# nacho-pancho/binary-image-compression

Measured on AMD Instinct MI355X. Metric: encode MPixels/s (and MB/s out) at 1/2/4/8 GPUs; bit-exact vs CPU, higher is better.
Workload: dtype u64; 1 GPU; c3: 16384x16384 8-bit gray -> 8 bitplanes -> med -> per-row runs -> Golomb + EG streams per plane (bitplanes formed in registers, not returned: planes NULL) -- the count pass writes the EG stream, the Golomb emission reads the residual rows from it; rows=16384, cols=16384, planes_per_gpu=8, parallelism=dp1 (independent images per GPU)

## Files before the change

binary-image-compression_amd/csrc/bic_kernels.hip:

```cpp
#include "bic_device.h"
#include "bic_k1pi.h"
#include "bic_kstat.h"

namespace bic {

__device__ __forceinline__ uint64_t transpose8x8(uint64_t x) {
  uint64_t t;
  t = (x ^ (x >> 7)) & 0x00AA00AA00AA00AAull;
  x = x ^ t ^ (t << 7);
  t = (x ^ (x >> 14)) & 0x0000CCCC0000CCCCull;
  x = x ^ t ^ (t << 14);
  t = (x ^ (x >> 28)) & 0x00000000F0F0F0F0ull;
  x = x ^ t ^ (t << 28);
  return x;
}

template <bool VEC, bool GC, int SP = 0>
__global__ __launch_bounds__(kBlock) void k_bitplanes_u8(const uint8_t* __restrict__ gray, size_t pitch,
                                                         uint32_t rows, uint32_t cols, uint32_t used,
                                                         int plane0, int nplanes, uint64_t* __restrict__ planes,
                                                         uint32_t wpr) {
  const uint32_t groups = (used + 63) / 64;
  const uint64_t gw = (uint64_t)blockIdx.x * kWaves + wave_id();
  if (gw >= (uint64_t)rows * groups) return;
// ... 206 lines not shown
  auto load = [&](uint32_t row, uint64_t (&v)[LW]) {
    const uint64_t* src = pl + (uint64_t)row * g.wpr + w0;
    if constexpr (LW == 1) {
      v[0] = w0 < g.used ? src[0] : 0;
    } else {
#pragma unroll
      for (int i = 0; i < LW; i += 2) {
        ulonglong2 t = make_ulonglong2(0, 0);
        if (w0 + i < g.used) t = *reinterpret_cast<const ulonglong2*>(src + i);
        v[i] = t.x;
        v[i + 1] = t.y;
      }
    }
  };
  uint64_t up[LW], cur[LW];
#pragma unroll
  for (int i = 0; i < LW; ++i) up[i] = 0;
  if (PREDICT && r0) load(r0 - 1, up);
  load(r0, cur);
  const uint32_t nr = min((uint32_t)RPW, g.rows - r0);
  for (uint32_t r = 0; r < nr; ++r) {
    const uint32_t row = r0 + r;
    uint64_t nxt[LW];
    if (r + 1 < nr) load(row + 1, nxt);
    LaneK k;
    uint64_t D[LW];
#pragma unroll
    for (int i = 0; i < LW; ++i) D[i] = PREDICT ? cur[i] ^ up[i] : cur[i];
    const uint64_t dl = wave_shr1_u64(D[LW - 1]);
#pragma unroll
    for (int i = 0; i < LW; ++i) {
      const uint32_t w = w0 + i;
      uint64_t R = D[i];
      if constexpr (PREDICT) {
        R = D[i] ^ ((D[i] >> 1) | ((i ? D[i - 1] : dl) << 63));
        if (row == 0 && w == 0) R &= ~BIC_MSB;
      }
      R = w < g.used ? (w == g.used - 1 ? R & g.trail : R) : 0;
      lanek_word(k, R, (int32_t)(w * 64));
      up[i] = cur[i];
    }
    const uint64_t id = (uint64_t)plane * g.rows + row;
    lanek_store(k, krec + id, kpos + id, sones + id);
#pragma unroll
    for (int i = 0; i < LW; ++i) cur[i] = nxt[i];
  }
}

template <int CTRL>
__device__ __forceinline__ int dpp16(int old, int v) {
  return __builtin_amdgcn_update_dpp(old, v, CTRL, 0xf, 0xf, false);
}
__device__ __forceinline__ uint32_t row16_incl_sum(uint32_t x) {
  x += (uint32_t)dpp16<0x111>(0, (int)x);
  x += (uint32_t)dpp16<0x112>(0, (int)x);
  x += (uint32_t)dpp16<0x114>(0, (int)x);
  x += (uint32_t)dpp16<0x118>(0, (int)x);
  return x;
}
__device__ __forceinline__ int row16_incl_max(int x) {
  x = max(x, dpp16<0x111>(INT_MIN, x));
  x = max(x, dpp16<0x112>(INT_MIN, x));
  x = max(x, dpp16<0x114>(INT_MIN, x));
  x = max(x, dpp16<0x118>(INT_MIN, x));
  return x;
}
__device__ __forceinline__ int row16_max(int x) {
  x = max(x, dpp16<0xB1>(x, x));
  x = max(x, dpp16<0x4E>(x, x));
  x = max(x, dpp16<0x141>(x, x));
  x = max(x, dpp16<0x140>(x, x));
  return x;
}
__device__ __forceinline__ int row16_min(int x) {
  x = min(x, dpp16<0xB1>(x, x));
  x = min(x, dpp16<0x4E>(x, x));
  x = min(x, dpp16<0x141>(x, x));
  x = min(x, dpp16<0x140>(x, x));
  return x;
}
__device__ __forceinline__ uint32_t row16_sum(uint32_t x) {
  x += (uint32_t)dpp16<0xB1>(0, (int)x);
  x += (uint32_t)dpp16<0x4E>(0, (int)x);
  x += (uint32_t)dpp16<0x141>(0, (int)x);
  x += (uint32_t)dpp16<0x140>(0, (int)x);
  return x;
}

template <int RPW, bool PREDICT, bool V16>
__global__ __launch_bounds__(kBlock) void k_med_kstat16(Geom g, const uint64_t* __restrict__ planes,
                                                        uint32_t* __restrict__ sones, int4* __restrict__ krec,
                                                        uint32_t* __restrict__ kpos, uint32_t* __restrict__ zero) {
  if (blockIdx.x == 0 && threadIdx.x < kZeroWords) zero[threadIdx.x] = 0;
  const int lane = lane_id(), q = lane & 15, grp = lane >> 4;
  const uint32_t wpp = (g.rows + RPW - 1) / RPW;
  const uint64_t gw = (uint64_t)xcd_remap(blockIdx.x, gridDim.x) * kWaves + wave_id();
  if (gw >= (uint64_t)wpp * g.nplanes) return;
  const uint32_t plane = (uint32_t)(gw / wpp), r0 = (uint32_t)(gw % wpp) * RPW;
  const uint64_t* pl = planes + (uint64_t)plane * g.plane_words;
  const uint32_t w0 = 4 * (uint32_t)q;
  const uint32_t nr = min((uint32_t)RPW, g.rows - r0);
  auto load = [&](uint32_t rb, uint64_t (&P)[4], uint64_t (&U)[4]) {
    const uint32_t rr = rb + (uint32_t)grp < nr ? r0 + rb + (uint32_t)grp : r0;
    if constexpr (V16) {
      const uint32_t wc = w0 < g.used ? w0 : 0;
      const ulonglong2* p2 = reinterpret_cast<const ulonglong2*>(pl + (uint64_t)rr * g.wpr + wc);
      const ulonglong2 a = p2[0], b = p2[1];
      P[0] = a.x; P[1] = a.y; P[2] = b.x; P[3] = b.y;
      if (PREDICT && rr) {
        const ulonglong2* u2 = reinterpret_cast<const ulonglong2*>(pl + (uint64_t)(rr - 1) * g.wpr + wc);
        const ulonglong2 c = u2[0], d = u2[1];
        U[0] = c.x; U[1] = c.y; U[2] = d.x; U[3] = d.y;
      } else {
        U[0] = U[1] = U[2] = U[3] = 0;
      }
      return;
    }
#pragma unroll
    for (int i = 0; i < 4; ++i) {
      const uint32_t w = w0 + i, wc = w < g.used ? w : g.used - 1;
      P[i] = pl[(uint64_t)rr * g.wpr + wc];
      U[i] = (PREDICT && rr) ? pl[(uint64_t)(rr - 1) * g.wpr + wc] : 0ull;
    }
  };
  uint64_t P[4], U[4];
  load(0, P, U);
  for (uint32_t rb = 0; rb < nr; rb += 4) {
    const uint32_t row = r0 + rb + (uint32_t)grp;
    const bool in = rb + (uint32_t)grp < nr;
    const uint32_t rr = in ? row : r0;
    uint64_t NP[4], NU[4];
    if (rb + 4 < nr) load(rb + 4, NP, NU);
    uint64_t D[4];
#pragma unroll
    for (int i = 0; i < 4; ++i) D[i] = P[i] ^ U[i];
    const uint64_t dl = ((uint64_t)(uint32_t)dpp16<0x111>(0, (int)(uint32_t)(D[3] >> 32)) << 32) |
                        (uint32_t)dpp16<0x111>(0, (int)(uint32_t)D[3]);
    LaneK k;
#pragma unroll
    for (int i = 0; i < 4; ++i) {
      const uint32_t w = w0 + i;
      uint64_t R = D[i];
      if constexpr (PREDICT) {
        R = D[i] ^ ((D[i] >> 1) | ((i ? D[i - 1] : dl) << 63));
        if (rr == 0 && w == 0) R &= ~BIC_MSB;
      }
      R = w < g.used ? (w == g.used - 1 ? R & g.trail : R) : 0;
      lanek_word(k, R, (int32_t)(w * 64));
    }
    const uint32_t inc = row16_incl_sum(k.ones);
    const int32_t base = (int32_t)(inc - k.ones);
    const int mx = row16_incl_max(k.last);
    const int32_t before = dpp16<0x111>(-1, mx);
    uint32_t chg = k.chg;
    int32_t first = -1;
    if (k.ones) {
      if (before >= 0) chg += (uint32_t)((before ^ k.first) & 1);
      else first = k.first;
    }
    const int32_t q0 = row16_max(k.ones ? k.q0 - 2 * base : -kNoOnes);
    const int32_t qh = row16_max(k.ones ? k.qh - 3 * base : -kNoOnes);
    const int32_t ql = row16_min(k.ones ? k.ql - 2 * base : kNoOnes);
    const uint32_t c = row16_sum(chg);
    const int32_t f = row16_max(first);
    const uint32_t tot = row16_sum(k.ones);
    const int32_t last = row16_max(k.last);
    if (q == 0 && in) {
      const uint64_t id = (uint64_t)plane * g.rows + row;
      krec[id] = make_int4(q0, qh, ql, (int32_t)(tot | (c << 16)));
      kpos[id] = ((uint32_t)f & 0xffffu) | ((uint32_t)last << 16);
      sones[id] = tot;
    }
#pragma unroll
    for (int i = 0; i < 4; ++i) {
      P[i] = NP[i];
      U[i] = NU[i];
    }
  }
}

void launch_row_ones(hipStream_t s, const Geom& g, const uint64_t* planes, int predict, uint32_t* sones,
                     int4* krec, uint32_t* kpos, uint32_t* zero) {
  constexpr int RPW = 8;
  const uint32_t wpp = (g.rows + RPW - 1) / RPW;
  const uint32_t grid = (uint32_t)(((uint64_t)wpp * g.nplanes + kWaves - 1) / kWaves);
#define BIC_KST(LW, P) k_med_kstat<LW, RPW, P><<<grid, kBlock, 0, s>>>(g, planes, sones, krec, kpos, zero)
  if (g.used <= 64) {
    constexpr int R16 = 16;
    const uint32_t wpp16 = (g.rows + R16 - 1) / R16;
    const uint32_t grid16 = (uint32_t)(((uint64_t)wpp16 * g.nplanes + kWaves - 1) / kWaves);
    const bool v16 = g.wpr % 4 == 0 && g.used % 4 == 0 && reinterpret_cast<uintptr_t>(planes) % 16 == 0;
#define BIC_K16(P, V) k_med_kstat16<R16, P, V><<<grid16, kBlock, 0, s>>>(g, planes, sones, krec, kpos, zero)
    if (predict) { if (v16) BIC_K16(true, true); else BIC_K16(true, false); }
    else { if (v16) BIC_K16(false, true); else BIC_K16(false, false); }
#undef BIC_K16
  }
  else if (g.used <= 128) { if (predict) BIC_KST(2, true); else BIC_KST(2, false); }
  else { if (predict) BIC_KST(4, true); else BIC_KST(4, false); }
#undef BIC_KST
}

template <int LW, int RPW, bool PREDICT>
__global__ __launch_bounds__(kBlock) void k_pbm_kstat(Geom g, const uint8_t* __restrict__ raster, uint64_t stride,
                                                      uint64_t* __restrict__ dst, int store_r,
                                                      uint32_t* __restrict__ sones, int4* __restrict__ krec,
                                                      uint32_t* __restrict__ kpos, uint32_t* __restrict__ zero) {
  static_assert(LW % 2 == 0, "a lane stores 16-byte word pairs");
  if (blockIdx.x == 0 && threadIdx.x < kZeroWords) zero[threadIdx.x] = 0;
  const int lane = lane_id();
  const uint32_t wpp = (g.rows + RPW - 1) / RPW;
  const uint64_t gw = (uint64_t)xcd_remap(blockIdx.x, gridDim.x) * kWaves + wave_id();
  if (gw >= (uint64_t)wpp * g.nplanes) return;
  const uint32_t plane = (uint32_t)(gw / wpp), r0 = (uint32_t)(gw % wpp) * RPW;
  const uint32_t nb = (g.cols + 7) / 8;
  const uint8_t* fp = raster + (uint64_t)plane * stride;
  const uint64_t fb = reinterpret_cast<uint64_t>(fp);
  const uint64_t lastc = (fb + (uint64_t)g.rows * nb - 1) & ~7ull;
  const uint32_t w0 = LW * lane;
  auto load = [&](uint32_t row, uint64_t (&v)[LW]) {
    const uint64_t a = fb + (uint64_t)row * nb + 8ull * w0;
    const uint32_t sh = 8 * (uint32_t)__builtin_amdgcn_readfirstlane((int)((fb + (uint64_t)row * nb) & 7));
    const uint64_t ca = a & ~7ull;
    uint64_t c[LW + 1];
#pragma unroll
    for (int j = 0; j <= LW; ++j) {
      const bool need = w0 + (j ? j - 1 : 0) < g.used && (j < LW || sh) && ca + 8 * j <= lastc;
      c[j] = need ? *reinterpret_cast<const uint64_t*>(fp + (int64_t)(ca + 8 * j - fb)) : 0ull;
    }
#pragma unroll
    for (int i = 0; i < LW; ++i) {
      const uint32_t w = w0 + i;
      const uint64_t x = bswap64(sh ? (c[i] >> sh) | (c[i + 1] << (64 - sh)) : c[i]);
      v[i] = w < g.used ? (w == g.used - 1 ? x & g.trail : x) : 0;
    }
  };
  uint64_t up[LW], cur[LW];
#pragma unroll
  for (int i = 0; i < LW; ++i) up[i] = 0;
  if (PREDICT && r0) load(r0 - 1, up);
  load(r0, cur);
  const uint32_t nr = min((uint32_t)RPW, g.rows - r0);
  uint64_t* out = dst + (uint64_t)plane * g.plane_words;
  for (uint32_t r = 0; r < nr; ++r) {
    const uint32_t row = r0 + r;
    uint64_t nxt[LW];
    if (r + 1 < nr) load(row + 1, nxt);
    LaneK k;
    uint64_t D[LW], R[LW];
#pragma unroll
    for (int i = 0; i < LW; ++i) D[i] = PREDICT ? cur[i] ^ up[i] : cur[i];
    const uint64_t dl = wave_shr1_u64(D[LW - 1]);
#pragma unroll
    for (int i = 0; i < LW; ++i) {
      const uint32_t w = w0 + i;
      R[i] = D[i];
      if constexpr (PREDICT) {
        R[i] = D[i] ^ ((D[i] >> 1) | ((i ? D[i - 1] : dl) << 63));
        if (row == 0 && w == 0) R[i] &= ~BIC_MSB;
      }
      R[i] = w < g.used ? (w == g.used - 1 ? R[i] & g.trail : R[i]) : 0;
      lanek_word(k, R[i], (int32_t)(w * 64));
      up[i] = cur[i];
    }
    const uint64_t id = (uint64_t)plane * g.rows + row;
    lanek_store(k, krec + id, kpos + id, sones + id);
    uint64_t* orow = out + (uint64_t)row * g.wpr;
#pragma unroll
    for (int i = 0; i < LW; i += 2)
      if (w0 + i < g.wpr)
        *reinterpret_cast<ulonglong2*>(orow + w0 + i) =
            store_r ? make_ulonglong2(R[i], R[i + 1]) : make_ulonglong2(cur[i], cur[i + 1]);
    for (uint32_t w = 64 * LW + 2 * lane; w < g.wpr; w += 128)
      *reinterpret_cast<ulonglong2*>(orow + w) = make_ulonglong2(0, 0);
#pragma unroll
    for (int i = 0; i < LW; ++i) cur[i] = nxt[i];
  }
}

void launch_pbm_rows(hipStream_t s, const uint8_t* raster, uint64_t stride, const Geom& g, int predict, uint64_t* dst,
                     bool store_resid, uint32_t* sones, int4* krec, uint32_t* kpos, uint32_t* zero) {
  constexpr int RPW = 8;
  const uint32_t wpp = (g.rows + RPW - 1) / RPW;
  const uint32_t grid = (uint32_t)(((uint64_t)wpp * g.nplanes + kWaves - 1) / kWaves);
  const int sr = store_resid && predict ? 1 : 0;
#define BIC_PKS(LW, P) k_pbm_kstat<LW, RPW, P><<<grid, kBlock, 0, s>>>(g, raster, stride, dst, sr, sones, krec, kpos, zero)
  if (g.used <= 128) { if (predict) BIC_PKS(2, true); else BIC_PKS(2, false); }
  else { if (predict) BIC_PKS(4, true); else BIC_PKS(4, false); }
#undef BIC_PKS
}

#ifndef BIC_GRAY_ROWS
#define BIC_GRAY_ROWS 4
#endif
#ifndef BIC_GRAY_ROWS_BM
#define BIC_GRAY_ROWS_BM 1
#endif
constexpr int kGrayRowsP = BIC_GRAY_ROWS, kGrayRowsBM = BIC_GRAY_ROWS_BM;
uint32_t gray_strips(const Geom& g) { return (g.used + 63) / 64; }

__device__ __forceinline__ void perm_t4(uint32_t w0, uint32_t w1, uint32_t w2, uint32_t w3, uint32_t (&out)[4]) {
  const uint32_t a01 = __builtin_amdgcn_perm(w0, w1, 0x04000501u), b01 = __builtin_amdgcn_perm(w0, w1, 0x06020703u);
  const uint32_t a23 = __builtin_amdgcn_perm(w2, w3, 0x04000501u), b23 = __builtin_amdgcn_perm(w2, w3, 0x06020703u);
  out[0] = __builtin_amdgcn_perm(a01, a23, 0x07060302u);
  out[1] = __builtin_amdgcn_perm(a01, a23, 0x05040100u);
  out[2] = __builtin_amdgcn_perm(b01, b23, 0x07060302u);
  out[3] = __builtin_amdgcn_perm(b01, b23, 0x05040100u);
}

__device__ __forceinline__ uint64_t transpose8x8_bs(uint32_t x0, uint32_t x1) {
  uint32_t hi = __builtin_bswap32(x0), lo = __builtin_bswap32(x1);
  uint32_t t;
  t = __builtin_amdgcn_bitop3_b32(lo, lo >> 7, 0x00AA00AAu, 0x28);
  lo = __builtin_amdgcn_bitop3_b32(lo, t, t << 7, 0x96);
  t = __builtin_amdgcn_bitop3_b32(hi, hi >> 7, 0x00AA00AAu, 0x28);
  hi = __builtin_amdgcn_bitop3_b32(hi, t, t << 7, 0x96);
  t = __builtin_amdgcn_bitop3_b32(lo, lo >> 14, 0x0000CCCCu, 0x28);
  lo = __builtin_amdgcn_bitop3_b32(lo, t, t << 14, 0x96);
  t = __builtin_amdgcn_bitop3_b32(hi, hi >> 14, 0x0000CCCCu, 0x28);
  hi = __builtin_amdgcn_bitop3_b32(hi, t, t << 14, 0x96);
  t = __builtin_amdgcn_bitop3_b32(lo, hi << 4, 0xF0F0F0F0u, 0x28);
  lo ^= t;
  hi ^= t >> 4;
  return ((uint64_t)hi << 32) | lo;
}

template <bool FULL = false>
__device__ __forceinline__ void gray_to_planes(const uint4 (&v)[4], uint64_t (&pw)[8], uint64_t mask) {
  uint64_t T[8];
#pragma unroll
  for (int i = 0; i < 4; ++i) {
    T[2 * i] = transpose8x8_bs(v[i].x, v[i].y);
    T[2 * i + 1] = transpose8x8_bs(v[i].z, v[i].w);
  }
  uint32_t XL[4], YL[4], XH[4], YH[4];
  perm_t4((uint32_t)T[0], (uint32_t)T[1], (uint32_t)T[2], (uint32_t)T[3], XL);
  perm_t4((uint32_t)T[4], (uint32_t)T[5], (uint32_t)T[6], (uint32_t)T[7], YL);
  perm_t4((uint32_t)(T[0] >> 32), (uint32_t)(T[1] >> 32), (uint32_t)(T[2] >> 32), (uint32_t)(T[3] >> 32), XH);
  perm_t4((uint32_t)(T[4] >> 32), (uint32_t)(T[5] >> 32), (uint32_t)(T[6] >> 32), (uint32_t)(T[7] >> 32), YH);
#pragma unroll
  for (int b = 0; b < 4; ++b) {
    pw[b] = ((uint64_t)XL[b] << 32) | YL[b];
    pw[4 + b] = ((uint64_t)XH[b] << 32) | YH[b];
    if constexpr (!FULL) {
      pw[b] &= mask;
      pw[4 + b] &= mask;
    }
  }
}

#ifndef BIC_GRAY_PREFETCH
#define BIC_GRAY_PREFETCH 1
#endif
constexpr bool kGrayPrefetch = BIC_GRAY_PREFETCH != 0;
#ifndef BIC_GRAY_BYTEMED
#define BIC_GRAY_BYTEMED 1
#endif
constexpr bool kGrayByteMed = BIC_GRAY_BYTEMED != 0;
template <bool PREDICT, bool STORE_R>
constexpr int gray_rows_per_wave() { return kGrayByteMed && PREDICT && STORE_R ? kGrayRowsBM : kGrayRowsP; }
__device__ __forceinline__ void load64_mis(const uint8_t* src, uint4 (&v)[4]) {
  const uintptr_t a = reinterpret_cast<uintptr_t>(src);
  const uint32_t mis = (uint32_t)(a & 15), bs = mis & 3, dq = mis >> 2;
  const uint4* b = reinterpret_cast<const uint4*>(src - mis);
  uint32_t in[20];
#pragma unroll
  for (int q = 0; q < 4; ++q) {
    const uint4 x = b[q];
    in[4 * q] = x.x;
    in[4 * q + 1] = x.y;
    in[4 * q + 2] = x.z;
    in[4 * q + 3] = x.w;
  }
  const uint4 x4 = mis ? b[4] : make_uint4(0, 0, 0, 0);
  in[16] = x4.x;
  in[17] = x4.y;
  in[18] = x4.z;
  in[19] = x4.w;
#define BIC_MIS_CASE(DQ)                                                                                    \
  case DQ:                                                                                                  \
    _Pragma("unroll") for (int q = 0; q < 4; ++q) v[q] =                                                    \
        make_uint4(__builtin_amdgcn_alignbyte(in[4 * q + DQ + 1], in[4 * q + DQ], bs),                     \
                   __builtin_amdgcn_alignbyte(in[4 * q + DQ + 2], in[4 * q + DQ + 1], bs),                 \
                   __builtin_amdgcn_alignbyte(in[4 * q + DQ + 3], in[4 * q + DQ + 2], bs),                 \
                   __builtin_amdgcn_alignbyte(in[4 * q + DQ + 4], in[4 * q + DQ + 3], bs));                \
    break;
  switch (dq) {
    BIC_MIS_CASE(0)
    BIC_MIS_CASE(1)
    BIC_MIS_CASE(2)
    default: BIC_MIS_CASE(3)
  }
#undef BIC_MIS_CASE
}

__device__ __forceinline__ void gray4(uint4 (&v)[4]) {
#pragma unroll
  for (int q = 0; q < 4; ++q)
    v[q] = make_uint4(v[q].x ^ ((v[q].x >> 1) & 0x7f7f7f7fu), v[q].y ^ ((v[q].y >> 1) & 0x7f7f7f7fu),
                      v[q].z ^ ((v[q].z >> 1) & 0x7f7f7f7fu), v[q].w ^ ((v[q].w >> 1) & 0x7f7f7f7fu));
}

struct Raw16 {
  uint4 cur[8], up[8];
};

template <bool PREDICT, bool FULL, bool STORE_R, bool NP8, bool EGS, bool MIS = false, int S16 = 0, bool GC = false,
          int CT = 0, int SP = 0>
__device__ __forceinline__ void gray_strip_rows(const uint8_t* __restrict__ gray, size_t pitch, const Geom& g,
                                                uint32_t ns, uint32_t s, uint32_t r0, uint32_t plane0,
                                                uint64_t* __restrict__ planes, uint32_t* __restrict__ sones,
                                                int4* __restrict__ krec, uint32_t* __restrict__ kpos, uint32_t* tw,
                                                uint64_t* __restrict__ out_e, uint64_t eg_stride, uint32_t bo = 0,
                                                const Raw16* pre = nullptr, uint32_t lo16 = 0) {
  const int lane = lane_id();
  const int np = NP8 ? 8 : (int)g.nplanes;
  const uint32_t w = s * 64 + lane;
  const bool in = FULL || w < g.used;
  const uint64_t mask = FULL ? ~0ull : in ? (w == g.used - 1 ? g.trail : ~0ull) : 0ull;
  auto load = [&](uint32_t row, uint4 (&v)[4], uint32_t& lb) {
    const uint8_t* src = gray + (uint64_t)row * pitch + (uint64_t)w * (S16 == 3 ? 192 : S16 ? 128 : 64);
    if constexpr (S16 == 3) {
      uint4 c[12];
      if (in) {
        if constexpr (MIS) {
#pragma unroll
          for (int t = 0; t < 3; ++t) {
            uint4 a[4];
            load64_mis(src + 64 * t, a);
#pragma unroll
            for (int q = 0; q < 4; ++q) c[4 * t + q] = a[q];
          }
        } else {
#pragma unroll
          for (int q = 0; q < 12; ++q) c[q] = reinterpret_cast<const uint4*>(src)[q];
        }
      } else {
#pragma unroll
        for (int q = 0; q < 12; ++q) c[q] = make_uint4(0, 0, 0, 0);
      }
      const uint32_t s1 = rgb_sel1(bo), s2 = rgb_sel2(bo);
      auto pick = [&](uint32_t d0, uint32_t d1, uint32_t d2) {
        uint32_t x = rgb_pick4(d0, d1, d2, s1, s2);
        if constexpr (CT != 0)
          if (bo != 1) x = ct_forward4<CT>(x, rgb_pick4(d0, d1, d2, rgb_sel1(1), rgb_sel2(1)));
        if constexpr (GC) x ^= (x >> 1) & 0x7f7f7f7fu;
        return x;
      };
#pragma unroll
      for (int q = 0; q < 4; ++q)
        v[q] = make_uint4(pick(c[3 * q].x, c[3 * q].y, c[3 * q].z), pick(c[3 * q].w, c[3 * q + 1].x, c[3 * q + 1].y),
                          pick(c[3 * q + 1].z, c[3 * q + 1].w, c[3 * q + 2].x),
                          pick(c[3 * q + 2].y, c[3 * q + 2].z, c[3 * q + 2].w));
    } else if constexpr (S16) {
      uint4 c[8];
      if constexpr (S16 == 2) {
#pragma unroll
        for (int q = 0; q < 8; ++q) c[q] = row == r0 ? pre->cur[q] : pre->up[q];
      } else if (in) {
        if constexpr (MIS) {
          uint4 a[4], b[4];
          load64_mis(src, a);
          load64_mis(src + 64, b);
#pragma unroll
          for (int q = 0; q < 4; ++q) c[q] = a[q], c[4 + q] = b[q];
        } else {
#pragma unroll
          for (int q = 0; q < 8; ++q) c[q] = reinterpret_cast<const uint4*>(src)[q];
        }
      } else {
#pragma unroll
        for (int q = 0; q < 8; ++q) c[q] = make_uint4(0, 0, 0, 0);
      }
      const uint32_t sel = bo ? 0x07050301u : 0x06040200u;
      auto pick = [&](uint32_t hi2, uint32_t lo2) {
        uint32_t x = __builtin_amdgcn_perm(hi2, lo2, sel);
        if constexpr (GC) {
          x ^= (x >> 1) & 0x7f7f7f7fu;
          if (lo16) x ^= (__builtin_amdgcn_perm(hi2, lo2, sel ^ 0x01010101u) & 0x01010101u) << 7;
        }
        return x;
      };
#pragma unroll
      for (int q = 0; q < 4; ++q)
        v[q] = make_uint4(pick(c[2 * q].y, c[2 * q].x), pick(c[2 * q].w, c[2 * q].z), pick(c[2 * q + 1].y, c[2 * q + 1].x),
                          pick(c[2 * q + 1].w, c[2 * q + 1].z));
    } else if constexpr (MIS) {
      if (in) load64_mis(src, v);
      else
#pragma unroll
        for (int q = 0; q < 4; ++q) v[q] = make_uint4(0, 0, 0, 0);
    } else {
#pragma unroll
      for (int q = 0; q < 4; ++q) v[q] = in ? reinterpret_cast<const uint4*>(src)[q] : make_uint4(0, 0, 0, 0);
    }
    if constexpr (S16 == 3) lb = (lane == 0 && s > 0) ? (uint32_t)src[(int)bo - 3] : 0u;
    else if constexpr (S16) lb = (lane == 0 && s > 0) ? (uint32_t)src[(int)bo - 2] : 0u;
    else lb = (lane == 0 && s > 0) ? (uint32_t)src[-1] : 0u;
    if constexpr (S16 == 3 && CT != 0)
      if (bo != 1 && lane == 0 && s > 0) lb = ct_forward4<CT>(lb, (uint32_t)src[-2]) & 0xffu;
    if constexpr (SP != 0) {
      static_assert(S16 == 0 || SP == 0, "sample prediction: one-byte gray samples only");
      uint32_t prev = (uint32_t)__builtin_amdgcn_update_dpp(0, (int)v[3].w, 0x138, 0xf, 0xf, true);
      if (lane == 0) prev = lb << 24;
#pragma unroll
      for (int q = 0; q < 4; ++q) {
        const uint4 x = v[q];
        v[q] = make_uint4(sp_forward4<SP>(x.x, prev), sp_forward4<SP>(x.y, x.x), sp_forward4<SP>(x.z, x.y),
                          sp_forward4<SP>(x.w, x.z));
        prev = x.w;
      }
      if (lane == 0 && s > 0) lb = ct_forward4<SP>(lb, (uint32_t)src[-2]) & 0xffu;
    }
    if constexpr (GC) {
      if constexpr (!S16) gray4(v);
      lb ^= lb >> 1;
      if constexpr (S16 == 1 || S16 == 2)
        if (lo16 && lane == 0 && s > 0) lb ^= ((uint32_t)src[(int)(bo ^ 1u) - 2] & 1u) << 7;
    }
    if (plane0) {
      const uint32_t m = 0x01010101u * (0xffu >> plane0);
#pragma unroll
      for (int q = 0; q < 4; ++q) v[q] = make_uint4((v[q].x >> plane0) & m, (v[q].y >> plane0) & m,
                                                    (v[q].z >> plane0) & m, (v[q].w >> plane0) & m);
      lb >>= plane0;
    }
  };
  constexpr bool BM = kGrayByteMed && PREDICT && STORE_R;
  constexpr bool PF = kGrayPrefetch && !(S16 == 3 && MIS);
  uint64_t up[8];
#pragma unroll
  for (int b = 0; b < 8; ++b) up[b] = 0;
  uint32_t ulast = 0, ulb = 0;
  uint4 cur[4], upb[4];
#pragma unroll
  for (int q = 0; q < 4; ++q) upb[q] = make_uint4(0, 0, 0, 0);
  uint32_t clb;
  if (PREDICT && r0) {
    load(r0 - 1, cur, ulb);
    if constexpr (BM) {
#pragma unroll
      for (int q = 0; q < 4; ++q) upb[q] = cur[q];
    } else {
      gray_to_planes<FULL>(cur, up, mask);
      ulast = cur[3].w >> 24;
    }
  }
  load(r0, cur, clb);
  const uint32_t nr = min((uint32_t)gray_rows_per_wave<PREDICT, STORE_R>(), g.rows - r0);
  for (uint32_t r = 0; r < nr; ++r) {
    const uint32_t row = r0 + r;
    uint4 nxt[4];
    uint32_t nlb = 0;
    if (PF && r + 1 < nr) load(row + 1, nxt, nlb);
    const bool lastS = s + 1 == ns;
    const uint32_t rn = lastS ? row + 1 : row;
    uint32_t gn = 0;
    if (EGS && FULL && rn < g.rows) {
      const uint8_t* cp = S16 == 3 ? gray + (uint64_t)rn * pitch + (lastS ? 0u : (s + 1) * 12288u) + 3 * lane + bo
                          : S16 ? gray + (uint64_t)rn * pitch + (lastS ? 0u : (s + 1) * 8192u) + 2 * lane + bo
                              : gray + (uint64_t)rn * pitch + (lastS ? 0u : (s + 1) * 4096u) + lane;
      uint32_t cb = cp[0], ub = rn ? cp[-(int64_t)pitch] : 0u;
      if constexpr (S16 == 3 && CT != 0)
        if (bo != 1) {
          const int64_t o = 1 - (int64_t)bo;
          cb = ct_forward4<CT>(cb, cp[o]) & 0xffu;
          if (rn) ub = ct_forward4<CT>(ub, cp[o - (int64_t)pitch]) & 0xffu;
        }
      if constexpr (SP != 0) {
        const bool nl = lastS && lane == 0;
        cb = ct_forward4<SP>(cb, nl ? 0u : (uint32_t)cp[-1]) & 0xffu;
        if (rn) ub = ct_forward4<SP>(ub, nl ? 0u : (uint32_t)cp[-1 - (int64_t)pitch]) & 0xffu;
      }
      uint32_t gd0 = cb ^ ub;
      if constexpr (GC) {
        gd0 ^= gd0 >> 1;
        if constexpr (S16 == 1 || S16 == 2)
          if (lo16) {
            const int64_t o = 1 - 2 * (int64_t)bo;
            const uint32_t co = cp[o], uo = rn ? cp[o - (int64_t)pitch] : 0u;
            gd0 ^= ((co ^ uo) & 1u) << 7;
          }
      }
      gn = gd0 >> plane0;
    }
    uint64_t pw[8];
    uint32_t left = 0;
    if constexpr (BM) {
      uint32_t gd[16];
#pragma unroll
      for (int q = 0; q < 4; ++q) {
        gd[4 * q] = cur[q].x ^ upb[q].x;
        gd[4 * q + 1] = cur[q].y ^ upb[q].y;
        gd[4 * q + 2] = cur[q].z ^ upb[q].z;
        gd[4 * q + 3] = cur[q].w ^ upb[q].w;
      }
      uint32_t gl = (uint32_t)__builtin_amdgcn_update_dpp(0, (int)(gd[15] >> 24), 0x138, 0xf, 0xf, true);
      if (lane == 0) gl = clb ^ ulb;
      uint32_t hd[16];
      hd[0] = gd[0] ^ __builtin_amdgcn_alignbyte(gd[0], gl << 24, 3);
#pragma unroll
      for (int d = 1; d < 16; ++d) hd[d] = gd[d] ^ __builtin_amdgcn_alignbyte(gd[d], gd[d - 1], 3);
      if (row == 0 && w == 0) hd[0] &= ~0xffu;
      if constexpr (EGS && FULL) {
        uint32_t gl2 = (uint32_t)__builtin_amdgcn_update_dpp(0, (int)gn, 0x138, 0xf, 0xf, true);
        if (lane == 0) gl2 = lastS ? 0u : (uint32_t)__builtin_amdgcn_readlane((int)gd[15], 63) >> 24;
        gn = (gn ^ gl2) & 0xffu;
      }
      uint4 hv[4];
#pragma unroll
      for (int q = 0; q < 4; ++q) hv[q] = make_uint4(hd[4 * q], hd[4 * q + 1], hd[4 * q + 2], hd[4 * q + 3]);
      gray_to_planes<FULL>(hv, pw, mask);
#pragma unroll
      for (int q = 0; q < 4; ++q) upb[q] = cur[q];
      ulb = clb;
    } else {
      const uint32_t cl = cur[3].w >> 24;
      const uint32_t dl = (PREDICT && row) ? cl ^ ulast : cl;
      left = (uint32_t)__builtin_amdgcn_update_dpp(0, (int)dl, 0x138, 0xf, 0xf, true);
      if (lane == 0) left = (PREDICT && row) ? clb ^ ulb : clb;
      ulast = cl;
      ulb = clb;
      gray_to_planes<FULL>(cur, pw, mask);
    }
    uint32_t* tb = tw;
    const uint64_t ep = (uint64_t)row * (g.cols + 1) + 1 + (uint64_t)s * 4096;
    const uint32_t esh = (uint32_t)(ep & 63);
    uint64_t* eo = out_e + (ep >> 6) + lane;
#pragma unroll
    for (int b = 0; b < 8; ++b) {
      if (!NP8 && b >= np) break;
      if (!STORE_R && in) planes[(uint64_t)b * g.plane_words + (uint64_t)row * g.wpr + w] = pw[b];
      uint64_t R = pw[b];
      if constexpr (PREDICT && !BM) {
        const uint64_t D = pw[b] ^ up[b];
        R = D ^ ((D >> 1) | ((uint64_t)((left >> b) & 1u) << 63));
        if constexpr (!FULL) R &= mask;
        if (row == 0 && w == 0) R &= ~BIC_MSB;
        up[b] = pw[b];
      }
      if (!EGS && STORE_R && in) planes[(uint64_t)b * g.plane_words + (uint64_t)row * g.wpr + w] = R;
      if constexpr (EGS && FULL) {
        const uint64_t E = ~R;
        uint64_t N = ~__builtin_bitreverse64(__ballot((gn >> b) & 1u));
        if (lastS) N = BIC_MSB | (rn < g.rows ? N >> 1 : 0ull);
        uint64_t* eb = eo + (uint64_t)b * eg_stride;
        if (esh == 0) {
          eb[0] = bswap64(E);
          if (lastS && lane == 63) eb[1] = bswap64(N);
        } else {
          uint64_t En = ((uint64_t)(uint32_t)__builtin_amdgcn_update_dpp(0, (int)(E >> 32), 0x130, 0xf, 0xf, true) << 32) |
                        (uint32_t)__builtin_amdgcn_update_dpp(0, (int)(uint32_t)E, 0x130, 0xf, 0xf, true);
          if (lane == 63) En = N;
          eb[1] = bswap64(funnel64(E, En, esh));
          if (row == 0 && s == 0 && lane == 0) eb[0] = bswap64(BIC_MSB | (E >> 1));
        }
      }
      strip_word_put(tb, b, R, (int32_t)(w * 64));
    }
    __builtin_amdgcn_fence(__ATOMIC_RELEASE, "wavefront");
    __builtin_amdgcn_wave_barrier();
    strip_records(tw, np, krec, kpos, sones, (uint64_t)row * ns + s, (uint64_t)g.rows * ns);
    __builtin_amdgcn_fence(__ATOMIC_ACQ_REL, "wavefront");
    __builtin_amdgcn_wave_barrier();
    if constexpr (PF) {
#pragma unroll
      for (int q = 0; q < 4; ++q) cur[q] = nxt[q];
      clb = nlb;
    } else if (r + 1 < nr) {
      load(row + 1, cur, clb);
    }
  }
}

#ifndef BIC_GRAY_WAVES
#define BIC_GRAY_WAVES 4
#endif
template <bool PREDICT, bool STORE_R, bool EGS, bool MIS = false, bool GC = false, int SP = 0>
__global__ __launch_bounds__(kBlock, BIC_GRAY_WAVES) void k_gray_strips(const uint8_t* __restrict__ gray, size_t pitch, Geom g,
                                                        uint32_t ns, uint32_t plane0, uint64_t* __restrict__ planes,
                                                        uint32_t* __restrict__ sones, int4* __restrict__ krec,
                                                        uint32_t* __restrict__ kpos, uint32_t* __restrict__ zero,
                                                        uint64_t* __restrict__ out_e, uint64_t eg_stride) {
  __shared__ __attribute__((aligned(16))) uint32_t tab[kWaves][1024];
  if (blockIdx.x == 0 && threadIdx.x < kZeroWords) zero[threadIdx.x] = 0;
  const uint32_t wv = wave_id();
  uint32_t* tw = tab[wv];
  const uint64_t gw = (uint64_t)xcd_remap(blockIdx.x, gridDim.x) * kWaves + wv;
  const uint32_t s = (uint32_t)(gw % ns);
  const uint32_t r0 = (uint32_t)(gw / ns) * gray_rows_per_wave<PREDICT, STORE_R>();
  if (r0 >= g.rows) return;
  if ((s + 1) * 64 <= g.used && g.trail == ~0ull && g.nplanes == 8)
    gray_strip_rows<PREDICT, true, STORE_R, true, EGS, MIS, 0, GC, 0, SP>(gray, pitch, g, ns, s, r0, plane0, planes, sones,
                                                                          krec, kpos, tw, out_e, eg_stride);
  else if ((s + 1) * 64 <= g.used && g.trail == ~0ull)
    gray_strip_rows<PREDICT, true, STORE_R, false, EGS, MIS, 0, GC, 0, SP>(gray, pitch, g, ns, s, r0, plane0, planes, sones,
                                                                           krec, kpos, tw, out_e, eg_stride);
  else if constexpr (!EGS)
    gray_strip_rows<PREDICT, false, STORE_R, false, false, MIS, 0, GC, 0, SP>(gray, pitch, g, ns, s, r0, plane0, planes,
                                                                              sones, krec, kpos, tw, nullptr, 0);
}

#ifndef BIC_GRAY16_BOTH
#define BIC_GRAY16_BOTH 1
#endif
constexpr bool kGray16Both = BIC_GRAY16_BOTH != 0 && kGrayByteMed && kGrayRowsBM == 1;
template <bool PREDICT, bool STORE_R, bool EGS, bool MIS = false, bool GC = false>
__global__ __launch_bounds__(kBlock, BIC_GRAY_WAVES) void k_gray_strips16(const uint8_t* __restrict__ gray, size_t pitch, Geom g,
                                                          uint32_t ns, uint32_t plane0, uint32_t be,
                                                          uint64_t* __restrict__ planes, uint32_t* __restrict__ sones,
                                                          int4* __restrict__ krec, uint32_t* __restrict__ kpos,
                                                          uint32_t* __restrict__ zero, uint64_t* __restrict__ out_e,
                                                          uint64_t eg_stride) {
  __shared__ __attribute__((aligned(16))) uint32_t tab[kWaves][1024];
  if (blockIdx.x == 0 && threadIdx.x < kZeroWords) zero[threadIdx.x] = 0;
  const uint32_t wv = wave_id();
  uint32_t* tw = tab[wv];
  const uint32_t nlo = plane0 < 8 ? min(8u, plane0 + g.nplanes) - plane0 : 0u, nhi = g.nplanes - nlo;
  const uint32_t ngrp = nlo && nhi ? 2u : 1u;
  constexpr bool BOTH = kGray16Both && PREDICT && STORE_R && !MIS;
  constexpr int S = BOTH ? 2 : 1;
  const uint32_t wgrp = BOTH ? 1u : ngrp;
  const uint64_t gw = (uint64_t)xcd_remap(blockIdx.x, gridDim.x) * kWaves + wv;
  const uint32_t hi = nlo ? (uint32_t)(gw % wgrp) : 1u;
  const uint64_t gs = gw / wgrp;
  const uint32_t s = (uint32_t)(gs % ns);
  const uint32_t r0 = (uint32_t)(gs / ns) * gray_rows_per_wave<PREDICT, STORE_R>();
  if (r0 >= g.rows) return;
  Raw16 raw;
  if constexpr (BOTH) {
    const uint32_t w = s * 64 + lane_id();
    const uint8_t* src = gray + (uint64_t)r0 * pitch + (uint64_t)w * 128;
    const bool in = w < g.used;
#pragma unroll
    for (int q = 0; q < 8; ++q) raw.cur[q] = raw.up[q] = make_uint4(0, 0, 0, 0);
    if (in) {
#pragma unroll
      for (int q = 0; q < 8; ++q) raw.cur[q] = reinterpret_cast<const uint4*>(src)[q];
    }
    if (in && r0) {
#pragma unroll
      for (int q = 0; q < 8; ++q) raw.up[q] = reinterpret_cast<const uint4*>(src - pitch)[q];
    }
  }
  auto group = [&](uint32_t h) __attribute__((always_inline)) {
    Geom gg = g;
    gg.nplanes = h ? nhi : nlo;
    const uint32_t p0 = h ? max(8u, plane0) - 8u : plane0;
    const uint32_t skip = h ? nlo : 0u;
    const uint32_t bo = h ^ (be ? 1u : 0u);
    const uint32_t lo16 = h ? 0u : 1u;
    const uint64_t rskip = (uint64_t)skip * g.rows * ns;
    uint64_t* pl = planes + (uint64_t)skip * g.plane_words;
    uint64_t* oe = out_e + (uint64_t)skip * eg_stride;
    if ((s + 1) * 64 <= g.used && g.trail == ~0ull && gg.nplanes == 8)
      gray_strip_rows<PREDICT, true, STORE_R, true, EGS, MIS, S, GC>(gray, pitch, gg, ns, s, r0, p0, pl, sones + rskip,
                                                                     krec + rskip, kpos + rskip, tw, oe, eg_stride, bo,
                                                                     &raw, lo16);
    else if ((s + 1) * 64 <= g.used && g.trail == ~0ull)
      gray_strip_rows<PREDICT, true, STORE_R, false, EGS, MIS, S, GC>(gray, pitch, gg, ns, s, r0, p0, pl, sones + rskip,
                                                                      krec + rskip, kpos + rskip, tw, oe, eg_stride, bo,
                                                                      &raw, lo16);
    else if constexpr (!EGS)
      gray_strip_rows<PREDICT, false, STORE_R, false, false, MIS, S, GC>(gray, pitch, gg, ns, s, r0, p0, pl,
                                                                         sones + rskip, krec + rskip, kpos + rskip, tw,
                                                                         nullptr, 0, bo, &raw, lo16);
  };
  if constexpr (BOTH) {
    if (nlo) group(0);
    if (nhi) group(1);
  } else {
    group(hi);
  }
}

template <bool PREDICT, bool STORE_R, bool EGS, bool MIS = false, bool GC = false, int CT = 0>
__global__ __launch_bounds__(kBlock, BIC_GRAY_WAVES) void k_gray_strips_rgb(const uint8_t* __restrict__ rgb, size_t pitch, Geom g,
                                                            uint32_t ns, uint32_t plane0, uint64_t* __restrict__ planes,
                                                            uint32_t* __restrict__ sones, int4* __restrict__ krec,
                                                            uint32_t* __restrict__ kpos, uint32_t* __restrict__ zero,
                                                            uint64_t* __restrict__ out_e, uint64_t eg_stride) {
  __shared__ __attribute__((aligned(16))) uint32_t tab[kWaves][1024];
  if (blockIdx.x == 0 && threadIdx.x < kZeroWords) zero[threadIdx.x] = 0;
  const uint32_t wv = wave_id();
  uint32_t* tw = tab[wv];
  const uint64_t gw = (uint64_t)xcd_remap(blockIdx.x, gridDim.x) * kWaves + wv;
  const uint32_t ch = (uint32_t)(gw % 3u);
  const uint64_t gs = gw / 3u;
  const uint32_t s = (uint32_t)(gs % ns);
  const uint32_t r0 = (uint32_t)(gs / ns) * gray_rows_per_wave<PREDICT, STORE_R>();
  if (r0 >= g.rows) return;
  Geom gg = g;
  gg.nplanes = g.nplanes / 3u;
  const uint32_t skip = ch * gg.nplanes;
  const uint64_t rskip = (uint64_t)skip * g.rows * ns;
  uint64_t* pl = planes + (uint64_t)skip * g.plane_words;
  uint64_t* oe = out_e + (uint64_t)skip * eg_stride;
  if ((s + 1) * 64 <= g.used && g.trail == ~0ull && gg.nplanes == 8)
    gray_strip_rows<PREDICT, true, STORE_R, true, EGS, MIS, 3, GC, CT>(rgb, pitch, gg, ns, s, r0, plane0, pl,
                                                                       sones + rskip, krec + rskip, kpos + rskip, tw,
                                                                       oe, eg_stride, ch);
  else if ((s + 1) * 64 <= g.used && g.trail == ~0ull)
    gray_strip_rows<PREDICT, true, STORE_R, false, EGS, MIS, 3, GC, CT>(rgb, pitch, gg, ns, s, r0, plane0, pl,
                                                                        sones + rskip, krec + rskip, kpos + rskip, tw,
                                                                        oe, eg_stride, ch);
  else if constexpr (!EGS)
// ... 1223 lines not shown
```

binary-image-compression_amd/csrc/bic_kstat.h:

```cpp
#pragma once
#include "bic_device.h"

namespace bic {

constexpr int32_t kNoOnes = 1 << 30;
constexpr uint32_t kMaxStrips = 4;

__device__ __forceinline__ uint32_t parity_changes(uint64_t x) {
  constexpr uint64_t kEven = 0xAAAAAAAAAAAAAAAAull;
  const uint64_t E = x & kEven, O = x & ~kEven;
  const uint64_t pe = (~x + (E << 1)) & x, po = (~x + (O << 1)) & x;
  return (uint32_t)__popcll(pe & O) + (uint32_t)__popcll(po & E);
}

struct LaneK {
  uint32_t ones = 0, chg = 0;
  int32_t q0 = -kNoOnes, qh = -kNoOnes, ql = kNoOnes, first = -1, last = -1;
};
__device__ __forceinline__ void lanek_word(LaneK& k, uint64_t x, int32_t c0) {
  if (!x) return;
  const int32_t m = __popcll(x), o = (int32_t)k.ones;
  const int32_t pl = c0 + 63 - __builtin_ctzll(x), pf = c0 + __builtin_clzll(x);
  k.q0 = max(k.q0, pl - m - 2 * o);
  k.qh = max(k.qh, pl - m - 3 * o - 1);
  k.ql = min(k.ql, pf - 2 * o - m);
  k.chg += parity_changes(x) + (k.last >= 0 ? (uint32_t)((k.last ^ pf) & 1) : 0u);
  if (k.first < 0) k.first = pf;
  k.last = pl;
  k.ones += m;
}

__device__ __forceinline__ void lanek_store(const LaneK& k, int4* rec, uint32_t* pos, uint32_t* sones) {
  if (__ballot(k.ones != 0) == ~0ull) {
    const int32_t before = dpp_or<0x138>(-1, k.last);
    const uint32_t chg = k.chg + (before >= 0 ? (uint32_t)((before ^ k.first) & 1) : 0u);
    const uint32_t inc = wave_incl_sum_u32(k.ones | (chg << 16));
    const int32_t base = (int32_t)((inc & 0xffffu) - k.ones);
    const int32_t q0 = wave_max(k.q0 - 2 * base);
    const int32_t qh = wave_max(k.qh - 3 * base);
    const int32_t ql = wave_min(k.ql - 2 * base);
    const uint32_t t = lane63_u32(inc), tot = t & 0xffffu;
    const uint32_t f = (uint32_t)__builtin_amdgcn_readlane(k.first, 0);
    const uint32_t last = lane63_u32((uint32_t)k.last);
    if (lane_id() == 0) {
      *rec = make_int4(q0, qh, ql, (int32_t)(tot | (t >> 16 << 16)));
      *pos = (f & 0xffffu) | (last << 16);
      *sones = tot;
    }
    return;
  }
  const uint32_t inc = wave_incl_sum_u32(k.ones);
  const int32_t base = (int32_t)(inc - k.ones);
  const int mx = wave_incl_max(k.last);
  const int32_t before = dpp_or<0x138>(-1, mx);
  uint32_t chg = k.chg;
  int32_t first = -1;
  if (k.ones) {
    if (before >= 0) chg += (uint32_t)((before ^ k.first) & 1);
    else first = k.first;
  }
  const int32_t q0 = wave_max(k.ones ? k.q0 - 2 * base : -kNoOnes);
  const int32_t qh = wave_max(k.ones ? k.qh - 3 * base : -kNoOnes);
  const int32_t ql = wave_min(k.ones ? k.ql - 2 * base : kNoOnes);
  const uint32_t c = wave_sum_u32(chg);
  const int32_t f = wave_max(first);
  const uint32_t tot = lane63_u32(inc);
  const uint32_t last = lane63_u32((uint32_t)mx);
  if (lane_id() == 0) {
    *rec = make_int4(q0, qh, ql, (int32_t)(tot | (c << 16)));
    *pos = ((uint32_t)f & 0xffffu) | (last << 16);
    *sones = tot;
  }
}

__device__ __forceinline__ void strip_word_put(uint32_t* t, int b, uint64_t x, int32_t c0) {
  const int lane = lane_id();
  const uint32_t m = (uint32_t)__popcll(x) | (parity_changes(x) << 8);
  uint32_t hh, hl, lh, ll;
  const uint32_t xh = (uint32_t)(x >> 32), xl = (uint32_t)x;
  asm volatile("v_ffbh_u32 %0, %1" : "=v"(hh) : "v"(xh));
  asm volatile("v_ffbh_u32 %0, %1" : "=v"(hl) : "v"(xl));
  asm volatile("v_ffbl_b32 %0, %1" : "=v"(lh) : "v"(xh));
  asm volatile("v_ffbl_b32 %0, %1" : "=v"(ll) : "v"(xl));
  const uint32_t lz = min(hh, hl + 32u), tz = min(ll, lh + 32u);
  const uint32_t c = ((uint32_t)c0 + lz) | (((uint32_t)c0 + 63u - tz) << 16);
  const uint32_t idx = ((uint32_t)(lane & 7) >> 2) * 256 + 32 * b + 4 * (lane >> 3) + (lane & 3);
  t[idx] = m;
  t[512 + idx] = c;
}
template <int CTRL>
__device__ __forceinline__ int dpp_same(int v) {
  return __builtin_amdgcn_mov_dpp(v, CTRL, 0xf, 0xf, true);
}
__device__ __forceinline__ void strip_records(const uint32_t* t, int np, int4* krec, uint32_t* kpos, uint32_t* sones,
                                              uint64_t id0, uint64_t pstride) {
  const int L = lane_id(), p = L >> 3, j = L & 7;
  const uint4 a0 = *reinterpret_cast<const uint4*>(t + 4 * L);
  const uint4 a1 = *reinterpret_cast<const uint4*>(t + 256 + 4 * L);
  const uint4 c0 = *reinterpret_cast<const uint4*>(t + 512 + 4 * L);
  const uint4 c1 = *reinterpret_cast<const uint4*>(t + 768 + 4 * L);
  const uint32_t av[8] = {a0.x, a0.y, a0.z, a0.w, a1.x, a1.y, a1.z, a1.w};
  const uint32_t cv[8] = {c0.x, c0.y, c0.z, c0.w, c1.x, c1.y, c1.z, c1.w};
  uint32_t ones = 0, chg = 0;
  int32_t first = -1, last = -1, q0 = -kNoOnes, qh = -kNoOnes, ql = kNoOnes;
#pragma unroll
  for (int i = 0; i < 8; ++i) {
    const int32_t m = (int32_t)(av[i] & 0xffu);
    if (m) {
      const int32_t pf = (int32_t)(cv[i] & 0xffffu), pl = (int32_t)(cv[i] >> 16), o = (int32_t)ones;
      chg += (av[i] >> 8) + (last >= 0 ? (uint32_t)((last ^ pf) & 1) : 0u);
      q0 = max(q0, pl - m - 2 * o);
      qh = max(qh, pl - m - 1 - 3 * o);
      ql = min(ql, pf - m - 2 * o);
      if (first < 0) first = pf;
      last = pl;
      ones += (uint32_t)m;
    }
  }
  uint32_t inc = ones;
  int32_t lmax = last;
#pragma unroll
  for (int d = 1; d < 8; d <<= 1) {
    const uint32_t o = d == 1 ? (uint32_t)dpp_or<0x111>(0, (int)inc) : d == 2 ? (uint32_t)dpp_or<0x112>(0, (int)inc)
                                                                             : (uint32_t)dpp_or<0x114>(0, (int)inc);
    const int32_t lm = d == 1 ? dpp_or<0x111>(-1, lmax) : d == 2 ? dpp_or<0x112>(-1, lmax) : dpp_or<0x114>(-1, lmax);
    if (j >= d) {
      inc += o;
      lmax = max(lmax, lm);
    }
  }
  const int32_t lprev = dpp_or<0x111>(-1, lmax);
  const int32_t before = j ? lprev : -1;
  const int32_t B = (int32_t)(inc - ones);
  if (ones) {
    if (before >= 0) chg += (uint32_t)((before ^ first) & 1);
    q0 -= 2 * B;
    qh -= 3 * B;
    ql -= 2 * B;
  }
  int32_t f = ones ? first : INT_MAX;
  uint32_t tot = ones;
#define BIC_RED8(CTRL)                          \
  q0 = max(q0, dpp_same<CTRL>(q0));             \
  qh = max(qh, dpp_same<CTRL>(qh));             \
  ql = min(ql, dpp_same<CTRL>(ql));             \
  f = min(f, dpp_same<CTRL>(f));                \
  last = max(last, dpp_same<CTRL>(last));       \
  chg += (uint32_t)dpp_same<CTRL>((int)chg);    \
  tot += (uint32_t)dpp_same<CTRL>((int)tot);
  BIC_RED8(0xB1)
  BIC_RED8(0x4E)
  BIC_RED8(0x141)
#undef BIC_RED8
  if (j == 0 && p < np) {
    const uint64_t id = id0 + (uint64_t)p * pstride;
    krec[id] = make_int4(q0, qh, ql, (int32_t)(tot | (chg << 16)));
    kpos[id] = ((uint32_t)(f == INT_MAX ? -1 : f) & 0xffffu) | ((uint32_t)last << 16);
    sones[id] = tot;
  }
}

struct RowK {
  int32_t q0, qh, ql;
  uint32_t ones, chg;
};
struct RowKRaw {
  int4 v[kMaxStrips];
  uint32_t pp[kMaxStrips];
};
__device__ __forceinline__ RowKRaw row_kstats_load(const int4* rec, const uint32_t* pos, uint32_t ns) {
  RowKRaw q;
#pragma unroll
  for (uint32_t s = 0; s < kMaxStrips; ++s) {
    q.v[s] = s < ns ? rec[s] : make_int4(0, 0, 0, 0);
    q.pp[s] = s < ns ? pos[s] : 0u;
  }
  return q;
}
__device__ __forceinline__ RowK row_kstats_combine(const RowKRaw& q, uint32_t cols) {
  const int4* v = q.v;
  const uint32_t* pp = q.pp;
  RowK r{0, 0, 0, 0, 0};
  int32_t last = -1;
#pragma unroll
  for (uint32_t s = 0; s < kMaxStrips; ++s) {
    const uint32_t o = (uint32_t)v[s].w & 0xffffu;
    if (!o) continue;
    r.q0 = max(r.q0, v[s].x - 2 * (int32_t)r.ones);
    r.qh = max(r.qh, v[s].y - 3 * (int32_t)r.ones);
    r.ql = min(r.ql, v[s].z - 2 * (int32_t)r.ones);
    r.chg += ((uint32_t)v[s].w >> 16) + (uint32_t)((last ^ (int32_t)(int16_t)(pp[s] & 0xffffu)) & 1);
    r.ones += o;
    last = (int16_t)(pp[s] >> 16);
  }
  r.chg += (uint32_t)((last ^ (int32_t)cols) & 1);
  return r;
}
__device__ __forceinline__ RowK row_kstats(const int4* rec, const uint32_t* pos, uint32_t ns, uint32_t cols) {
  return row_kstats_combine(row_kstats_load(rec, pos, ns), cols);
}

}
```

Measured before the change: 7.262 million MPix/s.

## Count only even-to-odd run parity changes and derive total via closed form

Replaces the per-word parity-change count (two popcounts over even and odd masks) with a single even-to-odd transition count. The full change count is reconstructed at row combine time as 2*(eo+join)+parity of cols, which relies on changes alternating. It also moves address computation for plane and EG stores into scalar registers with a per-lane offset, and injects lane 63's funnel word with v_writelane instead of a conditional select. The aim is fewer vector ALU ops in the hot count and emit loops, at the cost of depending on an algebraic identity that must stay bit-exact.

Result: no change. 7.354 million MPix/s, median of 6 (+1.3%).

```diff
diff --git a/binary-image-compression_amd/csrc/bic_kernels.hip b/binary-image-compression_amd/csrc/bic_kernels.hip
--- a/binary-image-compression_amd/csrc/bic_kernels.hip
+++ b/binary-image-compression_amd/csrc/bic_kernels.hip
@@ -382,16 +382,16 @@
     const int32_t base = (int32_t)(inc - k.ones);
     const int mx = row16_incl_max(k.last);
     const int32_t before = dpp16<0x111>(-1, mx);
-    uint32_t chg = k.chg;
+    uint32_t eo = k.eo;
     int32_t first = -1;
     if (k.ones) {
-      if (before >= 0) chg += (uint32_t)((before ^ k.first) & 1);
-      else first = k.first;
+      eo += eo_join(before, k.first);
+      if (before < 0) first = k.first;
     }
     const int32_t q0 = row16_max(k.ones ? k.q0 - 2 * base : -kNoOnes);
     const int32_t qh = row16_max(k.ones ? k.qh - 3 * base : -kNoOnes);
     const int32_t ql = row16_min(k.ones ? k.ql - 2 * base : kNoOnes);
-    const uint32_t c = row16_sum(chg);
+    const uint32_t c = row16_sum(eo);
     const int32_t f = row16_max(first);
     const uint32_t tot = row16_sum(k.ones);
     const int32_t last = row16_max(k.last);
@@ -578,6 +578,11 @@
   }
 }
 
+__device__ __forceinline__ uint32_t writelane63(uint32_t v, uint32_t s) {
+  asm("v_writelane_b32 %0, %1, 63" : "+v"(v) : "s"(s));
+  return v;
+}
+
 #ifndef BIC_GRAY_PREFETCH
 #define BIC_GRAY_PREFETCH 1
 #endif
@@ -776,7 +781,16 @@
     }
   }
   load(r0, cur, clb);
-  const uint32_t nr = min((uint32_t)gray_rows_per_wave<PREDICT, STORE_R>(), g.rows - r0);
+  constexpr uint32_t RPW = (uint32_t)gray_rows_per_wave<PREDICT, STORE_R>();
+  const uint32_t nr = RPW == 1 ? 1u : min(RPW, g.rows - r0);
+  const uint32_t lo8 = (uint32_t)lane * 8u;
+  typedef uint64_t __attribute__((address_space(1))) global_u64;
+  auto at_lane = [&](uint64_t* base, uint64_t woff) {
+    const uint64_t a = reinterpret_cast<uint64_t>(base + woff);
+    uint32_t alo = (uint32_t)a, ahi = (uint32_t)(a >> 32);
+    asm("" : "+s"(alo), "+s"(ahi));
+    return reinterpret_cast<global_u64*>((((uint64_t)ahi << 32) | alo) + lo8);
+  };
   for (uint32_t r = 0; r < nr; ++r) {
     const uint32_t row = r0 + r;
     uint4 nxt[4];
@@ -855,11 +869,11 @@
     uint32_t* tb = tw;
     const uint64_t ep = (uint64_t)row * (g.cols + 1) + 1 + (uint64_t)s * 4096;
     const uint32_t esh = (uint32_t)(ep & 63);
-    uint64_t* eo = out_e + (ep >> 6) + lane;
+    const uint64_t ew = ep >> 6, pw0 = (uint64_t)row * g.wpr + s * 64;
 #pragma unroll
     for (int b = 0; b < 8; ++b) {
       if (!NP8 && b >= np) break;
-      if (!STORE_R && in) planes[(uint64_t)b * g.plane_words + (uint64_t)row * g.wpr + w] = pw[b];
+      if (!STORE_R && in) *at_lane(planes, pw0 + (uint64_t)b * g.plane_words) = pw[b];
       uint64_t R = pw[b];
       if constexpr (PREDICT && !BM) {
         const uint64_t D = pw[b] ^ up[b];
@@ -868,19 +882,19 @@
         if (row == 0 && w == 0) R &= ~BIC_MSB;
         up[b] = pw[b];
       }
-      if (!EGS && STORE_R && in) planes[(uint64_t)b * g.plane_words + (uint64_t)row * g.wpr + w] = R;
+      if (!EGS && STORE_R && in) *at_lane(planes, pw0 + (uint64_t)b * g.plane_words) = R;
       if constexpr (EGS && FULL) {
         const uint64_t E = ~R;
         uint64_t N = ~__builtin_bitreverse64(__ballot((gn >> b) & 1u));
         if (lastS) N = BIC_MSB | (rn < g.rows ? N >> 1 : 0ull);
-        uint64_t* eb = eo + (uint64_t)b * eg_stride;
+        auto* eb = at_lane(out_e, ew + (uint64_t)b * eg_stride);
         if (esh == 0) {
           eb[0] = bswap64(E);
           if (lastS && lane == 63) eb[1] = bswap64(N);
         } else {
-          uint64_t En = ((uint64_t)(uint32_t)__builtin_amdgcn_update_dpp(0, (int)(E >> 32), 0x130, 0xf, 0xf, true) << 32) |
-                        (uint32_t)__builtin_amdgcn_update_dpp(0, (int)(uint32_t)E, 0x130, 0xf, 0xf, true);
-          if (lane == 63) En = N;
+          const uint32_t e1 = (uint32_t)__builtin_amdgcn_update_dpp(0, (int)(E >> 32), 0x130, 0xf, 0xf, true);
+          const uint32_t e0 = (uint32_t)__builtin_amdgcn_update_dpp(0, (int)(uint32_t)E, 0x130, 0xf, 0xf, true);
+          const uint64_t En = ((uint64_t)writelane63(e1, (uint32_t)(N >> 32)) << 32) | writelane63(e0, (uint32_t)N);
           eb[1] = bswap64(funnel64(E, En, esh));
           if (row == 0 && s == 0 && lane == 0) eb[0] = bswap64(BIC_MSB | (E >> 1));
         }
diff --git a/binary-image-compression_amd/csrc/bic_kstat.h b/binary-image-compression_amd/csrc/bic_kstat.h
--- a/binary-image-compression_amd/csrc/bic_kstat.h
+++ b/binary-image-compression_amd/csrc/bic_kstat.h
@@ -1,20 +1,14 @@
 #pragma once
 #include "bic_device.h"
+#include "bic_kstat_eo.h"
 
 namespace bic {
 
 constexpr int32_t kNoOnes = 1 << 30;
 constexpr uint32_t kMaxStrips = 4;
 
-__device__ __forceinline__ uint32_t parity_changes(uint64_t x) {
-  constexpr uint64_t kEven = 0xAAAAAAAAAAAAAAAAull;
-  const uint64_t E = x & kEven, O = x & ~kEven;
-  const uint64_t pe = (~x + (E << 1)) & x, po = (~x + (O << 1)) & x;
-  return (uint32_t)__popcll(pe & O) + (uint32_t)__popcll(po & E);
-}
-
 struct LaneK {
-  uint32_t ones = 0, chg = 0;
+  uint32_t ones = 0, eo = 0;
   int32_t q0 = -kNoOnes, qh = -kNoOnes, ql = kNoOnes, first = -1, last = -1;
 };
 __device__ __forceinline__ void lanek_word(LaneK& k, uint64_t x, int32_t c0) {
@@ -24,7 +18,7 @@
   k.q0 = max(k.q0, pl - m - 2 * o);
   k.qh = max(k.qh, pl - m - 3 * o - 1);
   k.ql = min(k.ql, pf - 2 * o - m);
-  k.chg += parity_changes(x) + (k.last >= 0 ? (uint32_t)((k.last ^ pf) & 1) : 0u);
+  k.eo += eo_word(x) + eo_join(k.last, pf);
   if (k.first < 0) k.first = pf;
   k.last = pl;
   k.ones += m;
@@ -33,8 +27,8 @@
 __device__ __forceinline__ void lanek_store(const LaneK& k, int4* rec, uint32_t* pos, uint32_t* sones) {
   if (__ballot(k.ones != 0) == ~0ull) {
     const int32_t before = dpp_or<0x138>(-1, k.last);
-    const uint32_t chg = k.chg + (before >= 0 ? (uint32_t)((before ^ k.first) & 1) : 0u);
-    const uint32_t inc = wave_incl_sum_u32(k.ones | (chg << 16));
+    const uint32_t eo = k.eo + eo_join(before, k.first);
+    const uint32_t inc = wave_incl_sum_u32(k.ones | (eo << 16));
     const int32_t base = (int32_t)((inc & 0xffffu) - k.ones);
     const int32_t q0 = wave_max(k.q0 - 2 * base);
     const int32_t qh = wave_max(k.qh - 3 * base);
@@ -53,16 +47,16 @@
   const int32_t base = (int32_t)(inc - k.ones);
   const int mx = wave_incl_max(k.last);
   const int32_t before = dpp_or<0x138>(-1, mx);
-  uint32_t chg = k.chg;
+  uint32_t eo = k.eo;
   int32_t first = -1;
   if (k.ones) {
-    if (before >= 0) chg += (uint32_t)((before ^ k.first) & 1);
-    else first = k.first;
+    eo += eo_join(before, k.first);
+    if (before < 0) first = k.first;
   }
   const int32_t q0 = wave_max(k.ones ? k.q0 - 2 * base : -kNoOnes);
   const int32_t qh = wave_max(k.ones ? k.qh - 3 * base : -kNoOnes);
   const int32_t ql = wave_min(k.ones ? k.ql - 2 * base : kNoOnes);
-  const uint32_t c = wave_sum_u32(chg);
+  const uint32_t c = wave_sum_u32(eo);
   const int32_t f = wave_max(first);
   const uint32_t tot = lane63_u32(inc);
   const uint32_t last = lane63_u32((uint32_t)mx);
@@ -75,7 +69,7 @@
 
 __device__ __forceinline__ void strip_word_put(uint32_t* t, int b, uint64_t x, int32_t c0) {
   const int lane = lane_id();
-  const uint32_t m = (uint32_t)__popcll(x) | (parity_changes(x) << 8);
+  const uint32_t m = (uint32_t)__popcll(x) | (eo_word(x) << 8);
   uint32_t hh, hl, lh, ll;
   const uint32_t xh = (uint32_t)(x >> 32), xl = (uint32_t)x;
   asm volatile("v_ffbh_u32 %0, %1" : "=v"(hh) : "v"(xh));
@@ -101,14 +95,14 @@
   const uint4 c1 = *reinterpret_cast<const uint4*>(t + 768 + 4 * L);
   const uint32_t av[8] = {a0.x, a0.y, a0.z, a0.w, a1.x, a1.y, a1.z, a1.w};
   const uint32_t cv[8] = {c0.x, c0.y, c0.z, c0.w, c1.x, c1.y, c1.z, c1.w};
-  uint32_t ones = 0, chg = 0;
+  uint32_t ones = 0, eo = 0;
   int32_t first = -1, last = -1, q0 = -kNoOnes, qh = -kNoOnes, ql = kNoOnes;
 #pragma unroll
   for (int i = 0; i < 8; ++i) {
     const int32_t m = (int32_t)(av[i] & 0xffu);
     if (m) {
       const int32_t pf = (int32_t)(cv[i] & 0xffffu), pl = (int32_t)(cv[i] >> 16), o = (int32_t)ones;
-      chg += (av[i] >> 8) + (last >= 0 ? (uint32_t)((last ^ pf) & 1) : 0u);
+      eo += (av[i] >> 8) + eo_join(last, pf);
       q0 = max(q0, pl - m - 2 * o);
       qh = max(qh, pl - m - 1 - 3 * o);
       ql = min(ql, pf - m - 2 * o);
@@ -133,7 +127,7 @@
   const int32_t before = j ? lprev : -1;
   const int32_t B = (int32_t)(inc - ones);
   if (ones) {
-    if (before >= 0) chg += (uint32_t)((before ^ first) & 1);
+    eo += eo_join(before, first);
     q0 -= 2 * B;
     qh -= 3 * B;
     ql -= 2 * B;
@@ -146,7 +140,7 @@
   ql = min(ql, dpp_same<CTRL>(ql));             \
   f = min(f, dpp_same<CTRL>(f));                \
   last = max(last, dpp_same<CTRL>(last));       \
-  chg += (uint32_t)dpp_same<CTRL>((int)chg);    \
+  eo += (uint32_t)dpp_same<CTRL>((int)eo);      \
   tot += (uint32_t)dpp_same<CTRL>((int)tot);
   BIC_RED8(0xB1)
   BIC_RED8(0x4E)
@@ -154,7 +148,7 @@
 #undef BIC_RED8
   if (j == 0 && p < np) {
     const uint64_t id = id0 + (uint64_t)p * pstride;
-    krec[id] = make_int4(q0, qh, ql, (int32_t)(tot | (chg << 16)));
+    krec[id] = make_int4(q0, qh, ql, (int32_t)(tot | (eo << 16)));
     kpos[id] = ((uint32_t)(f == INT_MAX ? -1 : f) & 0xffffu) | ((uint32_t)last << 16);
     sones[id] = tot;
   }
@@ -189,11 +183,11 @@
     r.q0 = max(r.q0, v[s].x - 2 * (int32_t)r.ones);
     r.qh = max(r.qh, v[s].y - 3 * (int32_t)r.ones);
     r.ql = min(r.ql, v[s].z - 2 * (int32_t)r.ones);
-    r.chg += ((uint32_t)v[s].w >> 16) + (uint32_t)((last ^ (int32_t)(int16_t)(pp[s] & 0xffffu)) & 1);
+    r.chg += ((uint32_t)v[s].w >> 16) + eo_join(last, (int32_t)(pp[s] & 0xffffu));
     r.ones += o;
     last = (int16_t)(pp[s] >> 16);
   }
-  r.chg += (uint32_t)((last ^ (int32_t)cols) & 1);
+  r.chg = eo_row_chg(r.chg, last, cols);
   return r;
 }
 __device__ __forceinline__ RowK row_kstats(const int4* rec, const uint32_t* pos, uint32_t ns, uint32_t cols) {
diff --git a/binary-image-compression_amd/csrc/bic_kstat_eo.h b/binary-image-compression_amd/csrc/bic_kstat_eo.h
--- /dev/null
+++ b/binary-image-compression_amd/csrc/bic_kstat_eo.h
@@ -0,0 +1,24 @@
+#pragma once
+#include <cstdint>
+#if defined(__HIPCC__)
+#include <hip/hip_runtime.h>
+#define BIC_EO_HDI __host__ __device__ __attribute__((always_inline)) inline
+#else
+#define BIC_EO_HDI __attribute__((always_inline)) inline
+#endif
+
+namespace bic {
+
+BIC_EO_HDI uint32_t eo_word(uint64_t x) {
+  constexpr uint64_t kEven = 0xAAAAAAAAAAAAAAAAull;
+  const uint64_t pred = (~x + ((x & ~kEven) << 1)) & x;
+  return (uint32_t)__builtin_popcountll(pred & kEven);
+}
+
+BIC_EO_HDI uint32_t eo_join(int32_t last, int32_t next) { return (uint32_t)(~last & next) & 1u; }
+
+BIC_EO_HDI uint32_t eo_row_chg(uint32_t eo, int32_t last, uint32_t cols) {
+  return 2u * (eo + eo_join(last, (int32_t)cols)) + (~cols & 1u);
+}
+
+}
```
